# INK-USC/RE-Net

Measured on NVIDIA B200. Metric: rgcn_aggregate_edge_messages_per_sec, higher is better.
Workload: dtype f32

## Files before the change

include/renet_b200.h:

```cpp
#ifndef RENET_B200_H
#define RENET_B200_H

#include <stdint.h>

#ifdef __cplusplus
extern "C" {
#endif

typedef enum {
  RENET_OK = 0,
  RENET_ERR_INVALID_ARG = -1,
  RENET_ERR_CUDA = -2,
  RENET_ERR_NO_DEVICE = -3
} renet_status;

int renet_version(void);
const char* renet_last_error(void);
int64_t renet_launch_count(void);

int renet_set_gemm_engine(int engine);
int renet_get_gemm_engine(void);
int renet_set_weight_generation(int64_t generation);
int renet_set_scratch(void* device_ptr, int64_t bytes);

// ... 12 lines not shown

int renet_selfloop_gemm(const float* H, const int32_t* h_index, const float* Wloop, float* Hout,
                        int64_t N, int32_t d_in, int32_t d_out, void* stream);
int renet_rgcn_gather(const float* H, const int32_t* h_index, const float* W,
                      const int32_t* row_ptr, const int32_t* col_src, const int32_t* col_type,
                      const float* norm, float* Hout,
                      int64_t N, int64_t E, int32_t d_in, int32_t d_out,
                      int32_t num_bases, int32_t R2, int32_t relu, int32_t has_loop, void* stream);
int renet_rgcn_gather_hot(const float* H, const int32_t* h_index, const float* W,
                          const int32_t* row_ptr, const int32_t* col_src, const int32_t* col_type,
                          const float* norm, float* Hout,
                          int64_t N, int64_t E, int32_t d_in, int32_t d_out,
                          int32_t num_bases, int32_t R2, int32_t relu, int32_t has_loop,
                          const int32_t* hot_rel, int32_t n_hot, void* stream);
int renet_debug_stream_timing(void* buffer);

int renet_rgcn_block_bwd(const float* H, const int32_t* h_index,
                         const float* W, const float* Wloop,
                         const int32_t* t_row_ptr, const int32_t* t_col_dst, const int32_t* t_col_type,
                         const int32_t* rel_ptr, const int32_t* rel_src, const int32_t* rel_dst,
                         const float* norm, const float* Hout, const float* dHout,
                         float* dH, float* dW, float* dWloop, float* G_ws,
                         int64_t N, int64_t E, int32_t d_in, int32_t d_out,
                         int32_t num_bases, int32_t R2, int32_t relu, void* stream);

int renet_rgcn_bipartite_bwd(const float* H, const float* W,
                             const int32_t* t_row_ptr, const int32_t* t_col_dst, const int32_t* t_col_type,
                             const int32_t* rel_ptr, const int32_t* rel_src, const int32_t* rel_dst,
                             const float* norm, const float* Hout, const float* dHout,
                             float* dH, float* dW, float* G_ws,
// ... 170 lines not shown
```

renet_b200/_lib.py:

```python
import ctypes
import os

import torch

_HERE = os.path.dirname(os.path.abspath(__file__))
LIB_PATH = os.path.join(_HERE, 'librenet_b200.so')

_vp, _i32, _i64 = ctypes.c_void_p, ctypes.c_int32, ctypes.c_int64

SIGNATURES = {
    'renet_version': (ctypes.c_int, []),
    'renet_last_error': (ctypes.c_char_p, []),
    'renet_launch_count': (_i64, []),
    'renet_set_gemm_engine': (ctypes.c_int, [ctypes.c_int]),
    'renet_get_gemm_engine': (ctypes.c_int, []),
    'renet_set_weight_generation': (ctypes.c_int, [_i64]),
    'renet_set_scratch': (ctypes.c_int, [_vp, _i64]),
    'renet_csr_workspace_bytes': (_i64, [_i64, _i64]),
    'renet_build_csr': (ctypes.c_int, [_vp, _vp, _vp, _i64, _i64, _vp, _vp, _vp, _vp, _vp, _i64, _vp]),
    'renet_rgcn_block_fwd': (ctypes.c_int, [_vp] * 9 + [_i64, _i64, _i32, _i32, _i32, _i32, _i32, _vp]),
    'renet_selfloop_gemm': (ctypes.c_int, [_vp, _vp, _vp, _vp, _i64, _i32, _i32, _vp]),
    'renet_selfloop_gemm_bwd': (ctypes.c_int, [_vp, _vp, _vp, _vp, _vp, _vp, _vp, _i64, _i32, _i32, _vp]),
    'renet_rgcn_gather': (ctypes.c_int, [_vp] * 8 + [_i64, _i64, _i32, _i32, _i32, _i32, _i32, _i32, _vp]),
    'renet_debug_stream_timing': (ctypes.c_int, [_vp]),
    'renet_rgcn_gather_hot': (ctypes.c_int, [_vp] * 8 + [_i64, _i64, _i32, _i32, _i32, _i32, _i32, _i32, _vp, _i32, _vp]),
    'renet_rgcn_block_bwd': (ctypes.c_int, [_vp] * 17 + [_i64, _i64, _i32, _i32, _i32, _i32, _i32, _vp]),
    'renet_rgcn_bipartite_bwd': (ctypes.c_int, [_vp] * 14 + [_i64, _i64, _i64, _i32, _i32, _i32, _i32, _i32, _vp]),
    'renet_readout_subgraph_workspace_bytes': (_i64, [_i64, _i64]),
    'renet_readout_subgraph': (ctypes.c_int, [_vp, _i64, _i64] + [_vp] * 12 + [_i64, _vp]),
    'renet_scatter_add_rows': (ctypes.c_int, [_vp, _vp, _vp, _i64, _i32, _vp]),
    'renet_gru_workspace_bytes': (_i64, [_i64, _i64, _i64, _i32]),
    'renet_gru_fwd': (ctypes.c_int, [_vp] * 11 + [_i32] + [_vp] * 10 + [_i64, _i64, _i64, _i32, _vp, _i64, _vp]),
    'renet_gru_bwd_workspace_bytes': (_i64, [_i64, _i64, _i64, _i32]),
    'renet_gru_bwd': (ctypes.c_int, [_vp] * 11 + [_i32] + [_vp] * 18 + [_i64, _i64, _i64, _i64, _i32, _vp, _vp, _i64, _vp]),
    'renet_gru_dropout_workspace_bytes': (_i64, [_i64, _i64, _i64, _i32]),
    'renet_gru_fwd_dropout': (ctypes.c_int, [_vp] * 12 + [_i32] + [_vp] * 10 + [_i64, _i64, _i64, _i32, ctypes.c_float, ctypes.c_uint64, _vp, _i64, _vp]),
    'renet_gru_bwd_dropout_workspace_bytes': (_i64, [_i64, _i64, _i64, _i32]),
    'renet_gru_bwd_dropout': (ctypes.c_int, [_vp] * 12 + [_i32] + [_vp] * 18 + [_i64, _i64, _i64, _i64, _i32, ctypes.c_float, ctypes.c_uint64, _vp, _vp, _i64, _vp]),
    'renet_dropout_mask': (ctypes.c_int, [ctypes.c_uint64, ctypes.c_uint64, _i64, ctypes.c_float, _vp, _vp]),
# ... 123 lines not shown
```

renet_b200/csrc/api.cu:

```cuda
#include <cub/device/device_radix_sort.cuh>

#include <atomic>
#include <string.h>

#include "common.cuh"

namespace renet {

static thread_local char g_err[512] = "";
static std::atomic<int64_t> g_launches{0};

void set_error(const char* fmt, ...) {
  va_list ap;
  va_start(ap, fmt);
  vsnprintf(g_err, sizeof(g_err), fmt, ap);
  va_end(ap);
}
void count_launch(int n) { g_launches.fetch_add(n, std::memory_order_relaxed); }

int launch_rgcn_gather(const float* H, const int32_t* h_index, const float* W, const int32_t* row_ptr,
                       const int32_t* col_src, const int32_t* col_type, const float* norm, float* Hout,
                       int64_t N, int64_t E, int d_in, int d_out, int nb, int relu, int has_loop,
                       cudaStream_t stream, int R2 = -1, const int32_t* hot_rel = nullptr, int n_hot = 0);
int launch_rgcn_bwd(const float* H, const int32_t* h_index, const float* W, const float* Wloop,
// ... 176 lines not shown
                          int64_t E, int32_t d_in, int32_t d_out, int32_t num_bases, int32_t R2, int32_t relu,
                          int32_t has_loop, const int32_t* hot_rel, int32_t n_hot, void* stream) {
  int rc = check_layer_args("renet_rgcn_gather_hot", H, W, row_ptr, norm, Hout, N, E, d_in, d_out, num_bases, R2);
  if (rc) return rc;
  RENET_CHECK_ARG(E == 0 || (col_src && col_type), "renet_rgcn_gather_hot: null edge arrays");
  RENET_CHECK_ARG(n_hot >= 0 && (n_hot == 0 || hot_rel != nullptr), "renet_rgcn_gather_hot: bad hot-relation list");
  return launch_rgcn_gather(H, h_index, W, row_ptr, col_src, col_type, norm, Hout, N, E, d_in, d_out, num_bases,
                            relu, has_loop, (cudaStream_t)stream, R2, n_hot > 0 ? hot_rel : nullptr, n_hot);
}

int renet_debug_stream_timing(void* buffer) {
  set_stream_debug_buffer(static_cast<long long*>(buffer));
  return RENET_OK;
}

int renet_rgcn_block_fwd(const float* H, const int32_t* h_index, const float* W, const float* Wloop,
                         const int32_t* row_ptr, const int32_t* col_src, const int32_t* col_type,
                         const float* norm, float* Hout, int64_t N, int64_t E, int32_t d_in, int32_t d_out,
                         int32_t num_bases, int32_t R2, int32_t relu, void* stream) {
  int rc = check_layer_args("renet_rgcn_block_fwd", H, W, row_ptr, norm, Hout, N, E, d_in, d_out, num_bases, R2);
  if (rc) return rc;
  RENET_CHECK_ARG(E == 0 || (col_src && col_type), "renet_rgcn_block_fwd: null edge arrays");
  if (N == 0) return RENET_OK;
  if (Wloop != nullptr) {
    rc = sgemm_nn(H, h_index, d_in, Wloop, d_out, Hout, d_out, nullptr, N, d_out, d_in, false, (cudaStream_t)stream);
    if (rc) return rc;
  }
  return launch_rgcn_gather(H, h_index, W, row_ptr, col_src, col_type, norm, Hout, N, E, d_in, d_out, num_bases,
                            relu, Wloop != nullptr, (cudaStream_t)stream, R2);
}
// ... 307 lines not shown
```

renet_b200/csrc/common.cuh:

```cuda
#pragma once
#include <cuda_runtime.h>
#include <stdint.h>
#include <stdio.h>
#include <stdarg.h>

#include "../../include/renet_b200.h"

namespace renet {

void set_error(const char* fmt, ...);
void count_launch(int n = 1);

#define RENET_CHECK_ARG(cond, ...)                  \
  do {                                              \
    if (!(cond)) {                                  \
      ::renet::set_error(__VA_ARGS__);              \
      return RENET_ERR_INVALID_ARG;                 \
    }                                               \
  } while (0)

#define RENET_CHECK_CUDA(expr)                                                        \
  do {                                                                                \
    cudaError_t _e = (expr);                                                          \
    if (_e != cudaSuccess) {                                                          \
// ... 34 lines not shown
}

int sgemm_nn(const float* A, const int32_t* a_index, int64_t lda, const float* B, int64_t ldb, float* C,
             int64_t ldc, const float* bias, int64_t M, int32_t N, int32_t K, bool accumulate,
             cudaStream_t stream);
int sgemm_tn(const float* A, const int32_t* a_index, int64_t lda, const float* B, int64_t ldb, float* C,
             int64_t ldc, int32_t M, int32_t N, int64_t K, bool accumulate, cudaStream_t stream);
int sgemm_nt(const float* A, int64_t lda, const float* B, int64_t ldb, float* C, int64_t ldc,
             int64_t M, int32_t N, int32_t K, bool accumulate, cudaStream_t stream);

int gather_kernel_choice();
constexpr int64_t kStreamMinEdges = 16384;
constexpr int64_t kStreamMinNodes = 16384;
constexpr int64_t kStreamMaxNodes = 98304;
bool gather_use_stream(int64_t E, int64_t N);
void set_stream_debug_buffer(long long* p);

int gemm_mode();
int64_t umma_packed_bytes(int N, int K);
void set_weight_generation(int64_t g);
void* packed_cache_lookup(const void* const* keys, int nkeys, int64_t bytes, bool* hit);
bool umma_shape_ok(int N, int K);
int umma_pack_b(const float* B, int64_t sk, int64_t sn, int N, int K, void* Bp, int tile_offset, cudaStream_t stream);
struct EpiArgs {
  const int32_t* target;
  const float* lse;
  float* pmax;
  float* psum;
  float* tlogit;
  float* dT;
// ... 14 lines not shown
```

renet_b200/csrc/umma_gemm.cu:

```cuda
#include "common.cuh"
#include <mutex>
#include <vector>

#include "umma.cuh"

namespace renet {
namespace {

constexpr int UM = 128;
constexpr int UN = 200;
constexpr int UNP = 208;
constexpr int UKC = 40;
constexpr int USLABS = UKC / 4;
constexpr int UTHREADS = 256;
constexpr int A_SLAB_BYTES = UM * 16;
constexpr int B_SLAB_BYTES = UNP * 16;
constexpr int A_BYTES = USLABS * A_SLAB_BYTES;
constexpr int B_BYTES = USLABS * B_SLAB_BYTES;
constexpr int STAGE_BYTES = 2 * A_BYTES + 2 * B_BYTES;
constexpr int NUM_STAGES = 2;
constexpr int SMEM_BYTES = NUM_STAGES * STAGE_BYTES + 64;
constexpr int TMEM_COLS = 256;

__device__ __forceinline__ uint32_t make_idesc() { return make_idesc_n(UNP); }
// ... 154 lines not shown
  if (warp == 0) {
    asm volatile("tcgen05.dealloc.cta_group::1.sync.aligned.b32 %0, %1;" ::"r"(tmem_base), "n"(TMEM_COLS) : "memory");
  }
}


constexpr int P_BK = 32;
constexpr int P_A_BYTES = UM * 128;
constexpr int P_B_BYTES = UNP * 128;
constexpr int P_B_CHUNK = 2 * P_B_BYTES;
constexpr int P_SMEM = 4 * P_A_BYTES + 2 * P_B_CHUNK + 1024 + 128;

__global__ void __launch_bounds__(256)
umma_pack_b_kernel(const float* __restrict__ B, int64_t sk, int64_t sn, int N, int K, uint8_t* __restrict__ Bp,
                   int n_chunks, int tile_offset) {
  const int nt = blockIdx.x, kc = blockIdx.y;
  const int n0 = nt * UN, k0 = kc * P_BK;
  const int tile_n = min(UN, N - n0);
  uint8_t* dst = Bp + (size_t)((nt + tile_offset) * n_chunks + kc) * P_B_CHUNK;
  for (int task = blockIdx.z * 256 + threadIdx.x; task < UNP * 8; task += 256 * gridDim.z) {
    const int j = task / UNP, n = task % UNP;
    float v[4];
#pragma unroll
    for (int i = 0; i < 4; ++i) {
      const int k = k0 + 4 * j + i;
      v[i] = (n < tile_n && k < K) ? __ldg(B + (int64_t)k * sk + (int64_t)(n0 + n) * sn) : 0.f;
    }
    float4 hi, lo;
    split4(make_float4(v[0], v[1], v[2], v[3]), hi, lo);
    const uint32_t off = sw128_offset(n, j);
// ... 232 lines not shown
  }
  asm volatile("tcgen05.fence::before_thread_sync;" ::: "memory");
  __syncthreads();
  if (warp == 0) {
    asm volatile("tcgen05.dealloc.cta_group::1.sync.aligned.b32 %0, %1;" ::"r"(tmem_base), "n"(512) : "memory");
  }
}

constexpr int SL_PROD_WARPS = 8;
constexpr int SL_PROD = SL_PROD_WARPS * 32;
constexpr int SL_TMA_WARP = 8;
constexpr int SL_MMA_WARP = 9;
constexpr int SL_EPI_WARP0 = 10;
constexpr int SL_THREADS = (SL_EPI_WARP0 + 4) * 32;
constexpr int SL_A_STAGES = 3;
constexpr int SL_B_STAGES = 2;
constexpr int SL_A_STAGE = 2 * P_A_BYTES;
constexpr int SL_EPI_LD = 36;
constexpr int SL_EPI_WARP_BYTES = 32 * SL_EPI_LD * 4;
constexpr int SL_OFF_B = SL_A_STAGES * SL_A_STAGE;
constexpr int SL_OFF_EPI = SL_OFF_B + SL_B_STAGES * P_B_CHUNK;
constexpr int SL_OFF_BAR = SL_OFF_EPI + 4 * SL_EPI_WARP_BYTES;
constexpr int SL_SMEM = SL_OFF_BAR + 128 + 1024;
constexpr int SL_HALF0_N = 112;
static_assert(SL_SMEM <= 227 * 1024, "self-loop kernel: shared memory budget");
static_assert((SL_HALF0_N * 128) % 1024 == 0, "column half must start on a swizzle atom");
constexpr int SL_BAR_A_FULL = 0, SL_BAR_A_EMPTY = 3, SL_BAR_B_FULL = 6, SL_BAR_B_EMPTY = 8, SL_BAR_T_FULL = 10,
              SL_BAR_T_EMPTY = 12, SL_NUM_BARS = 14;

struct SlUnit {
  int64_t row0;
  int col0;
  int n;
};
__device__ __forceinline__ SlUnit sl_unit(int u, int split) {
  SlUnit s;
  if (split) {
    s.row0 = (int64_t)(u >> 1) * UM;
    s.col0 = (u & 1) ? SL_HALF0_N : 0;
    s.n = (u & 1) ? UNP - SL_HALF0_N : SL_HALF0_N;
  } else {
    s.row0 = (int64_t)u * UM;
    s.col0 = 0;
    s.n = UNP;
  }
  return s;
}

template <bool INDEXED>
__global__ void __launch_bounds__(SL_THREADS, 1)
umma_selfloop_kernel(const float* __restrict__ A, const int32_t* __restrict__ a_index, int64_t lda,
                     const uint8_t* __restrict__ Bp, float* __restrict__ C, int64_t ldc, int64_t M, int K, int n_chunks,
                     int n_units, int split) {
  extern __shared__ uint8_t smem_raw[];
  const uint32_t raw = smem_u32(smem_raw);
  uint8_t* smem = smem_raw + ((1024 - (raw & 1023)) & 1023);
  const int tid = threadIdx.x, warp = tid >> 5, lane = tid & 31;
  const uint32_t smem_base = smem_u32(smem);
  const uint32_t bar0 = smem_base + SL_OFF_BAR;
  auto bar = [&](int i) { return bar0 + 8 * i; };
  uint32_t* tmem_slot = reinterpret_cast<uint32_t*>(smem + SL_OFF_BAR + 8 * SL_NUM_BARS);

  if (tid == 0) {
    for (int s = 0; s < SL_A_STAGES; ++s) {
      mbar_init(bar(SL_BAR_A_FULL + s), SL_PROD);
      mbar_init(bar(SL_BAR_A_EMPTY + s), 1);
    }
    for (int s = 0; s < SL_B_STAGES; ++s) {
      mbar_init(bar(SL_BAR_B_FULL + s), 1);
      mbar_init(bar(SL_BAR_B_EMPTY + s), 1);
    }
    for (int a = 0; a < 2; ++a) {
      mbar_init(bar(SL_BAR_T_FULL + a), 1);
      mbar_init(bar(SL_BAR_T_EMPTY + a), 128);
    }
    asm volatile("fence.mbarrier_init.release.cluster;" ::: "memory");
  }
  if (warp == SL_MMA_WARP) {
    asm volatile("tcgen05.alloc.cta_group::1.sync.aligned.shared::cta.b32 [%0], %1;" ::"r"(smem_u32(tmem_slot)), "n"(512)
                 : "memory");
    asm volatile("tcgen05.relinquish_alloc_permit.cta_group::1.sync.aligned;" ::: "memory");
  }
  asm volatile("tcgen05.fence::before_thread_sync;" ::: "memory");
  __syncthreads();
  asm volatile("tcgen05.fence::after_thread_sync;" ::: "memory");
  const uint32_t tmem_base = *tmem_slot;

  const int n_local = (n_units - (int)blockIdx.x + (int)gridDim.x - 1) / (int)gridDim.x;
  const int total = n_local * n_chunks;
  const int last_ks = (K - (n_chunks - 1) * P_BK + 7) / 8;

  if (warp < SL_PROD_WARPS) {
    const int j = tid & 7;
    uint32_t a_off[4];
#pragma unroll
    for (int t = 0; t < 4; ++t) a_off[t] = sw128_offset((tid >> 3) + 32 * t, j);
    const float* rows[4];
    float4 vnext[4];
    auto set_rows = [&](int lu) {
      const SlUnit un = sl_unit((int)blockIdx.x + lu * (int)gridDim.x, split);
#pragma unroll
      for (int t = 0; t < 4; ++t) {
        const int64_t gr = un.row0 + (tid >> 3) + 32 * t;
        rows[t] = nullptr;
        if (gr < M) rows[t] = A + (INDEXED ? (int64_t)__ldg(a_index + gr) : gr) * lda;
      }
    };
    auto load = [&](int c) {
      const int k = c * P_BK + 4 * j;
#pragma unroll
      for (int t = 0; t < 4; ++t) {
        vnext[t] = make_float4(0.f, 0.f, 0.f, 0.f);
        if (rows[t] != nullptr && k < K) vnext[t] = ldg_f4(rows[t] + k);
      }
    };
    set_rows(0);
    load(0);
    for (int it = 0; it < total; ++it) {
      const int s = it % SL_A_STAGES, round = it / SL_A_STAGES;
      float4 v[4];
#pragma unroll
      for (int t = 0; t < 4; ++t) v[t] = vnext[t];
      if (it + 1 < total) {
        const int lu = (it + 1) / n_chunks, c = it + 1 - lu * n_chunks;
        if (c == 0) set_rows(lu);
        load(c);
      }
      if (round > 0) mbar_wait(bar(SL_BAR_A_EMPTY + s), (round - 1) & 1);
      uint8_t* sA_hi = smem + s * SL_A_STAGE;
      uint8_t* sA_lo = sA_hi + P_A_BYTES;
#pragma unroll
      for (int t = 0; t < 4; ++t) {
        float4 hi, lo;
        split4(v[t], hi, lo);
        *reinterpret_cast<float4*>(sA_hi + a_off[t]) = hi;
        *reinterpret_cast<float4*>(sA_lo + a_off[t]) = lo;
      }
      asm volatile("fence.proxy.async.shared::cta;" ::: "memory");
      asm volatile("mbarrier.arrive.shared::cta.b64 _, [%0];" ::"r"(bar(SL_BAR_A_FULL + s)) : "memory");
    }
  } else if (warp == SL_TMA_WARP) {
    if (lane == 0) {
      for (int it = 0; it < total; ++it) {
        const int s = it % SL_B_STAGES, round = it / SL_B_STAGES;
        const int lu = it / n_chunks, c = it - lu * n_chunks;
        const SlUnit un = sl_unit((int)blockIdx.x + lu * (int)gridDim.x, split);
        if (round > 0) mbar_wait(bar(SL_BAR_B_EMPTY + s), (round - 1) & 1);
        const uint32_t full = bar(SL_BAR_B_FULL + s);
        const uint32_t dst = smem_base + SL_OFF_B + s * P_B_CHUNK;
        const uint8_t* src = Bp + (size_t)c * P_B_CHUNK + un.col0 * 128;
        const uint32_t plane = (uint32_t)un.n * 128;
        asm volatile("mbarrier.arrive.expect_tx.shared::cta.b64 _, [%0], %1;" ::"r"(full), "r"(2 * plane) : "memory");
        if (un.n == UNP) {
          asm volatile("cp.async.bulk.shared::cluster.global.mbarrier::complete_tx::bytes [%0], [%1], %2, [%3];" ::"r"(dst),
                       "l"(src), "r"((uint32_t)P_B_CHUNK), "r"(full)
                       : "memory");
        } else {
#pragma unroll
          for (int p = 0; p < 2; ++p)
            asm volatile("cp.async.bulk.shared::cluster.global.mbarrier::complete_tx::bytes [%0], [%1], %2, [%3];" ::"r"(
                             dst + p * P_B_BYTES),
                         "l"(src + p * P_B_BYTES), "r"(plane), "r"(full)
                         : "memory");
        }
      }
    }
    __syncwarp();
  } else if (warp == SL_MMA_WARP) {
    if (lane == 0) {
      int it = 0;
      for (int lu = 0; lu < n_local; ++lu) {
        const int acc = lu & 1;
        const SlUnit un = sl_unit((int)blockIdx.x + lu * (int)gridDim.x, split);
        const uint32_t idesc = make_idesc_n(un.n);
        if (lu >= 2) mbar_wait(bar(SL_BAR_T_EMPTY + acc), ((lu >> 1) - 1) & 1);
        asm volatile("tcgen05.fence::after_thread_sync;" ::: "memory");
        const uint32_t d = tmem_base + acc * 256;
        for (int c = 0; c < n_chunks; ++c, ++it) {
          const int sa = it % SL_A_STAGES, sb = it % SL_B_STAGES;
          mbar_wait(bar(SL_BAR_A_FULL + sa), (it / SL_A_STAGES) & 1);
          mbar_wait(bar(SL_BAR_B_FULL + sb), (it / SL_B_STAGES) & 1);
          asm volatile("tcgen05.fence::after_thread_sync;" ::: "memory");
          const uint32_t a_hi = smem_base + sa * SL_A_STAGE, a_lo = a_hi + P_A_BYTES;
          const uint32_t b_hi = smem_base + SL_OFF_B + sb * P_B_CHUNK, b_lo = b_hi + P_B_BYTES;
          const int nks = (c == n_chunks - 1) ? last_ks : P_BK / 8;
          for (int ks = 0; ks < nks; ++ks) {
            const uint32_t ko = ks * 32;
            const uint64_t dAh = make_desc_sw128(a_hi + ko), dAl = make_desc_sw128(a_lo + ko);
            const uint64_t dBh = make_desc_sw128(b_hi + ko), dBl = make_desc_sw128(b_lo + ko);
            umma_tf32(d, dAh, dBh, idesc, (c | ks) != 0);
            umma_tf32(d, dAl, dBh, idesc, 1);
            umma_tf32(d, dAh, dBl, idesc, 1);
          }
          umma_commit(bar(SL_BAR_A_EMPTY + sa));
          umma_commit(bar(SL_BAR_B_EMPTY + sb));
        }
        umma_commit(bar(SL_BAR_T_FULL + acc));
      }
    }
    __syncwarp();
  } else {
    const int q = warp & 3;
    float* stg = reinterpret_cast<float*>(smem + SL_OFF_EPI + (warp - SL_EPI_WARP0) * SL_EPI_WARP_BYTES);
    for (int lu = 0; lu < n_local; ++lu) {
      const int acc = lu & 1;
      const SlUnit un = sl_unit((int)blockIdx.x + lu * (int)gridDim.x, split);
      const int col_end = min(UN, un.col0 + un.n);
      const int nblk = (un.n + 31) / 32;
      mbar_wait(bar(SL_BAR_T_FULL + acc), (lu >> 1) & 1);
      asm volatile("tcgen05.fence::after_thread_sync;" ::: "memory");
      const uint32_t taddr = tmem_base + acc * 256 + ((uint32_t)(q * 32) << 16);
#pragma unroll 1
      for (int blk = 0; blk < nblk; ++blk) {
        uint32_t v[32];
        asm volatile(
            "tcgen05.ld.sync.aligned.32x32b.x32.b32 "
            "{%0,%1,%2,%3,%4,%5,%6,%7,%8,%9,%10,%11,%12,%13,%14,%15,%16,%17,%18,%19,%20,%21,%22,%23,%24,%25,%26,%27,%28,%29,%30,%31}, [%32];"
            : "=r"(v[0]), "=r"(v[1]), "=r"(v[2]), "=r"(v[3]), "=r"(v[4]), "=r"(v[5]), "=r"(v[6]), "=r"(v[7]), "=r"(v[8]),
              "=r"(v[9]), "=r"(v[10]), "=r"(v[11]), "=r"(v[12]), "=r"(v[13]), "=r"(v[14]), "=r"(v[15]), "=r"(v[16]),
              "=r"(v[17]), "=r"(v[18]), "=r"(v[19]), "=r"(v[20]), "=r"(v[21]), "=r"(v[22]), "=r"(v[23]), "=r"(v[24]),
              "=r"(v[25]), "=r"(v[26]), "=r"(v[27]), "=r"(v[28]), "=r"(v[29]), "=r"(v[30]), "=r"(v[31])
            : "r"(taddr + (uint32_t)(blk * 32)));
        asm volatile("tcgen05.wait::ld.sync.aligned;" ::: "memory");
        if (blk == nblk - 1) {
          asm volatile("tcgen05.fence::before_thread_sync;" ::: "memory");
          asm volatile("mbarrier.arrive.shared::cta.b64 _, [%0];" ::"r"(bar(SL_BAR_T_EMPTY + acc)) : "memory");
        }
#pragma unroll
        for (int i = 0; i < 8; ++i)
          *reinterpret_cast<uint4*>(stg + lane * SL_EPI_LD + 4 * i) = make_uint4(v[4 * i], v[4 * i + 1], v[4 * i + 2], v[4 * i + 3]);
        __syncwarp();
#pragma unroll
        for (int p = 0; p < 8; ++p) {
          const int r = 4 * p + (lane >> 3), c4 = lane & 7;
          const int64_t gr = un.row0 + q * 32 + r;
          const int gc = un.col0 + blk * 32 + 4 * c4;
          if (gr < M && gc < col_end) st_f4(C + gr * ldc + gc, *reinterpret_cast<const float4*>(stg + r * SL_EPI_LD + 4 * c4));
        }
        __syncwarp();
      }
    }
  }
  asm volatile("tcgen05.fence::before_thread_sync;" ::: "memory");
  __syncthreads();
  if (warp == SL_MMA_WARP) {
    asm volatile("tcgen05.dealloc.cta_group::1.sync.aligned.b32 %0, %1;" ::"r"(tmem_base), "n"(512) : "memory");
  }
}

}

static uint8_t* g_scratch = nullptr;
static int64_t g_scratch_bytes = 0;
void set_scratch(void* p, int64_t bytes) { g_scratch = (uint8_t*)p; g_scratch_bytes = p ? bytes : 0; }

namespace {
struct PackEntry {
  int device;
  const void* keys[6];
  int nkeys;
  int64_t bytes;
  void* buf;
  int64_t gen;
};
std::mutex g_pack_mu;
std::vector<PackEntry> g_pack_entries;
int64_t g_weight_generation = -1;
}

// ... 70 lines not shown
#undef RENET_UMMA_LAUNCH
  RENET_CHECK_LAUNCH("umma_gemm_packed_kernel");
  return k_splits;
}

int umma_gemm_prepacked(const float* A, const int32_t* a_index, int64_t lda, const void* Bp, float* C, int64_t ldc,
                        const float* bias, int64_t M, int N, int K, bool accumulate, int batch, int64_t batch_a,
                        int64_t batch_bp, int64_t batch_c, cudaStream_t stream) {
  EpiArgs none{};
  const int r = umma_gemm_prepacked_ex(A, a_index, lda, Bp, C, ldc, bias, M, N, K, accumulate, batch, batch_a, batch_bp, batch_c,
                                       0, none, 1, 0, stream);
  return r < 0 ? r : RENET_OK;
}

static int umma_selfloop(const float* A, const int32_t* a_index, int64_t lda, const void* Bp, float* C, int64_t ldc,
                         int64_t M, int K, cudaStream_t stream) {
  static bool attr = false;
  if (!attr) {
    RENET_CHECK_CUDA(cudaFuncSetAttribute(umma_selfloop_kernel<true>, cudaFuncAttributeMaxDynamicSharedMemorySize, SL_SMEM));
    RENET_CHECK_CUDA(cudaFuncSetAttribute(umma_selfloop_kernel<false>, cudaFuncAttributeMaxDynamicSharedMemorySize, SL_SMEM));
    attr = true;
  }
  static int sm_count[64] = {0};
  int dev = 0;
  RENET_CHECK_CUDA(cudaGetDevice(&dev));
  if (dev < 0 || dev >= 64) dev = 0;
  if (sm_count[dev] == 0) RENET_CHECK_CUDA(cudaDeviceGetAttribute(&sm_count[dev], cudaDevAttrMultiProcessorCount, dev));
  const int sms = sm_count[dev];
  const int64_t tiles = (M + UM - 1) / UM;
  const int split = 2 * tiles <= sms ? 1 : 0;
  const int64_t units = split ? 2 * tiles : tiles;
  RENET_CHECK_ARG(units < (int64_t)1 << 30, "umma_selfloop: too many rows");
  const int grid = (int)(units < sms ? units : sms);
  const int n_chunks = (K + P_BK - 1) / P_BK;
  if (a_index)
    umma_selfloop_kernel<true><<<grid, SL_THREADS, SL_SMEM, stream>>>(A, a_index, lda, (const uint8_t*)Bp, C, ldc, M, K,
                                                                     n_chunks, (int)units, split);
  else
    umma_selfloop_kernel<false><<<grid, SL_THREADS, SL_SMEM, stream>>>(A, a_index, lda, (const uint8_t*)Bp, C, ldc, M, K,
                                                                      n_chunks, (int)units, split);
  RENET_CHECK_LAUNCH("umma_selfloop_kernel");
  return RENET_OK;
}

int umma_gemm_nn_try(const float* A, const int32_t* a_index, int64_t lda, const float* B, int64_t ldb, float* C,
                     int64_t ldc, const float* bias, int64_t M, int32_t N, int32_t K, bool accumulate,
                     cudaStream_t stream) {
  const bool aligned = ((reinterpret_cast<uintptr_t>(A) | reinterpret_cast<uintptr_t>(B) | reinterpret_cast<uintptr_t>(C) |
                         reinterpret_cast<uintptr_t>(bias)) & 15) == 0;
  if (aligned && umma_shape_ok(N, K) && (lda % 4 == 0) && (ldc % 4 == 0) && M >= 64 && g_scratch != nullptr &&
      umma_packed_bytes(N, K) <= g_scratch_bytes && (reinterpret_cast<uintptr_t>(g_scratch) & 127) == 0) {
    bool hit = false;
    const void* keys[4] = {B, reinterpret_cast<const void*>((intptr_t)ldb), reinterpret_cast<const void*>((intptr_t)N),
                           reinterpret_cast<const void*>((intptr_t)K)};
    void* cached = packed_cache_lookup(keys, 4, umma_packed_bytes(N, K), &hit);
    void* Bp = cached ? cached : g_scratch;
    int rc = hit ? 0 : umma_pack_b(B, ldb, 1, N, K, Bp, 0, stream);
    if (rc) return rc;
    if (gemm_mode() == 1 && N == UN && K == UN && bias == nullptr && !accumulate)
      rc = umma_selfloop(A, a_index, lda, Bp, C, ldc, M, K, stream);
    else
      rc = umma_gemm_prepacked(A, a_index, lda, Bp, C, ldc, bias, M, N, K, accumulate, 1, 0, 0, 0, stream);
    return rc ? rc : 1;
  }
  const bool ok = (K % UKC == 0) && K >= UKC && (N % 8 == 0) && (lda % 4 == 0) && (ldb % 4 == 0) && (ldc % 4 == 0) &&
                  M >= 64 && aligned;
  if (!ok) return 0;
  static bool attr_set = false;
  if (!attr_set) {
    cudaError_t e1 = cudaFuncSetAttribute(umma_gemm_nn_kernel<true>, cudaFuncAttributeMaxDynamicSharedMemorySize, SMEM_BYTES);
    cudaError_t e2 = cudaFuncSetAttribute(umma_gemm_nn_kernel<false>, cudaFuncAttributeMaxDynamicSharedMemorySize, SMEM_BYTES);
    if (e1 != cudaSuccess || e2 != cudaSuccess) {
      set_error("cudaFuncSetAttribute(umma_gemm_nn_kernel) failed: %s", cudaGetErrorString(e1 != cudaSuccess ? e1 : e2));
      return RENET_ERR_CUDA;
    }
// ... 18 lines not shown
```

Baseline: 3.809 billion.

## Run self-loop UMMA GEMM as 2-CTA clusters with split B loads and PDL

Converts the self-loop tf32 GEMM kernel to cta_group::2 MMAs over CTA pairs in a cluster. Each CTA loads half of the B columns, and the leader issues the paired MMAs after a peer-ready barrier, so a pair covers a 256-row tile with shared B traffic. It also deepens the B pipeline to four stages, double-buffers the A register prefetch, and adds programmatic dependent launch after the weight pack kernel. Optional per-block timing instrumentation is included. The trade-offs are cross-CTA synchronization cost and fewer work units when M is small.

```diff
diff --git a/include/renet_b200.h b/include/renet_b200.h
--- a/include/renet_b200.h
+++ b/include/renet_b200.h
@@ -50,6 +50,7 @@
                           int32_t num_bases, int32_t R2, int32_t relu, int32_t has_loop,
                           const int32_t* hot_rel, int32_t n_hot, void* stream);
 int renet_debug_stream_timing(void* buffer);
+int renet_debug_selfloop_timing(void* buffer);
 
 int renet_rgcn_block_bwd(const float* H, const int32_t* h_index,
                          const float* W, const float* Wloop,
diff --git a/renet_b200/_lib.py b/renet_b200/_lib.py
--- a/renet_b200/_lib.py
+++ b/renet_b200/_lib.py
@@ -23,6 +23,7 @@
     'renet_selfloop_gemm_bwd': (ctypes.c_int, [_vp, _vp, _vp, _vp, _vp, _vp, _vp, _i64, _i32, _i32, _vp]),
     'renet_rgcn_gather': (ctypes.c_int, [_vp] * 8 + [_i64, _i64, _i32, _i32, _i32, _i32, _i32, _i32, _vp]),
     'renet_debug_stream_timing': (ctypes.c_int, [_vp]),
+    'renet_debug_selfloop_timing': (ctypes.c_int, [_vp]),
     'renet_rgcn_gather_hot': (ctypes.c_int, [_vp] * 8 + [_i64, _i64, _i32, _i32, _i32, _i32, _i32, _i32, _vp, _i32, _vp]),
     'renet_rgcn_block_bwd': (ctypes.c_int, [_vp] * 17 + [_i64, _i64, _i32, _i32, _i32, _i32, _i32, _vp]),
     'renet_rgcn_bipartite_bwd': (ctypes.c_int, [_vp] * 14 + [_i64, _i64, _i64, _i32, _i32, _i32, _i32, _i32, _vp]),
diff --git a/renet_b200/csrc/api.cu b/renet_b200/csrc/api.cu
--- a/renet_b200/csrc/api.cu
+++ b/renet_b200/csrc/api.cu
@@ -214,6 +214,11 @@
   return RENET_OK;
 }
 
+int renet_debug_selfloop_timing(void* buffer) {
+  set_selfloop_debug_buffer(static_cast<long long*>(buffer));
+  return RENET_OK;
+}
+
 int renet_rgcn_block_fwd(const float* H, const int32_t* h_index, const float* W, const float* Wloop,
                          const int32_t* row_ptr, const int32_t* col_src, const int32_t* col_type,
                          const float* norm, float* Hout, int64_t N, int64_t E, int32_t d_in, int32_t d_out,
diff --git a/renet_b200/csrc/common.cuh b/renet_b200/csrc/common.cuh
--- a/renet_b200/csrc/common.cuh
+++ b/renet_b200/csrc/common.cuh
@@ -72,6 +72,7 @@
 constexpr int64_t kStreamMinNodes = 16384;
 constexpr int64_t kStreamMaxNodes = 98304;
 bool gather_use_stream(int64_t E, int64_t N);
+void set_selfloop_debug_buffer(long long* p);
 void set_stream_debug_buffer(long long* p);
 
 int gemm_mode();
diff --git a/renet_b200/csrc/umma_gemm.cu b/renet_b200/csrc/umma_gemm.cu
--- a/renet_b200/csrc/umma_gemm.cu
+++ b/renet_b200/csrc/umma_gemm.cu
@@ -192,6 +192,7 @@
 __global__ void __launch_bounds__(256)
 umma_pack_b_kernel(const float* __restrict__ B, int64_t sk, int64_t sn, int N, int K, uint8_t* __restrict__ Bp,
                    int n_chunks, int tile_offset) {
+  asm volatile("griddepcontrol.launch_dependents;" ::: "memory");
   const int nt = blockIdx.x, kc = blockIdx.y;
   const int n0 = nt * UN, k0 = kc * P_BK;
   const int tile_n = min(UN, N - n0);
@@ -454,45 +455,128 @@
 constexpr int SL_EPI_WARP0 = 10;
 constexpr int SL_THREADS = (SL_EPI_WARP0 + 4) * 32;
 constexpr int SL_A_STAGES = 3;
-constexpr int SL_B_STAGES = 2;
+constexpr int SL_B_STAGES = 4;
 constexpr int SL_A_STAGE = 2 * P_A_BYTES;
+constexpr int SL_B_PLANE = (UNP / 2) * 128;
+constexpr int SL_B_STAGE = 2 * SL_B_PLANE;
 constexpr int SL_EPI_LD = 36;
 constexpr int SL_EPI_WARP_BYTES = 32 * SL_EPI_LD * 4;
 constexpr int SL_OFF_B = SL_A_STAGES * SL_A_STAGE;
-constexpr int SL_OFF_EPI = SL_OFF_B + SL_B_STAGES * P_B_CHUNK;
+constexpr int SL_OFF_EPI = SL_OFF_B + SL_B_STAGES * SL_B_STAGE;
 constexpr int SL_OFF_BAR = SL_OFF_EPI + 4 * SL_EPI_WARP_BYTES;
-constexpr int SL_SMEM = SL_OFF_BAR + 128 + 1024;
+constexpr int SL_SMEM = SL_OFF_BAR + 256 + 1024;
 constexpr int SL_HALF0_N = 112;
 static_assert(SL_SMEM <= 227 * 1024, "self-loop kernel: shared memory budget");
-static_assert((SL_HALF0_N * 128) % 1024 == 0, "column half must start on a swizzle atom");
-constexpr int SL_BAR_A_FULL = 0, SL_BAR_A_EMPTY = 3, SL_BAR_B_FULL = 6, SL_BAR_B_EMPTY = 8, SL_BAR_T_FULL = 10,
-              SL_BAR_T_EMPTY = 12, SL_NUM_BARS = 14;
+static_assert((SL_HALF0_N * 128) % 1024 == 0 && (SL_HALF0_N / 2 * 128) % 1024 == 0 && ((UNP - SL_HALF0_N) / 2 * 128) % 1024 == 0 &&
+                  (UNP / 2 * 128) % 1024 == 0,
+              "every CTA's share of a column range must start on a swizzle atom");
+constexpr int SL_BAR_A_FULL = 0, SL_BAR_A_EMPTY = 3, SL_BAR_B_FULL = 6, SL_BAR_B_EMPTY = 10, SL_BAR_T_FULL = 14,
+              SL_BAR_T_EMPTY = 16, SL_BAR_PEER_FULL = 18, SL_PEER_SLOTS = 4, SL_NUM_BARS = 22;
+static_assert(SL_PEER_SLOTS > SL_A_STAGES, "the peer runs at most SL_A_STAGES items ahead of the leader");
+static_assert(8 * SL_NUM_BARS + 4 <= 256, "barrier area");
 
 struct SlUnit {
   int64_t row0;
   int col0;
   int n;
 };
-__device__ __forceinline__ SlUnit sl_unit(int u, int split) {
+__device__ __forceinline__ SlUnit sl_unit(int u, int split, int rank) {
   SlUnit s;
-  if (split) {
-    s.row0 = (int64_t)(u >> 1) * UM;
-    s.col0 = (u & 1) ? SL_HALF0_N : 0;
-    s.n = (u & 1) ? UNP - SL_HALF0_N : SL_HALF0_N;
-  } else {
-    s.row0 = (int64_t)u * UM;
-    s.col0 = 0;
-    s.n = UNP;
-  }
+  const int64_t pair_row = split ? (u >> 1) : u;
+  s.row0 = pair_row * (2 * UM) + rank * UM;
+  s.col0 = (split && (u & 1)) ? SL_HALF0_N : 0;
+  s.n = split ? ((u & 1) ? UNP - SL_HALF0_N : SL_HALF0_N) : UNP;
   return s;
+}
+
+__device__ __forceinline__ uint32_t sl_cluster_rank() {
+  uint32_t r;
+  asm volatile("mov.u32 %0, %%cluster_ctarank;" : "=r"(r));
+  return r;
+}
+__device__ __forceinline__ uint32_t sl_mapa(uint32_t saddr, uint32_t rank) {
+  uint32_t r;
+  asm volatile("mapa.shared::cluster.u32 %0, %1, %2;" : "=r"(r) : "r"(saddr), "r"(rank));
+  return r;
+}
+__device__ __forceinline__ void sl_arrive_cluster(uint32_t cluster_addr) {
+  asm volatile("mbarrier.arrive.release.cluster.shared::cluster.b64 _, [%0];" ::"r"(cluster_addr) : "memory");
+}
+__device__ __forceinline__ void sl_cluster_sync() {
+  asm volatile("barrier.cluster.arrive.release.aligned;\n\tbarrier.cluster.wait.acquire.aligned;" ::: "memory");
+}
+__device__ __forceinline__ void sl_wait_cluster(uint32_t bar, uint32_t parity) {
+  uint32_t done = 0;
+  for (int spins = 0; !done; ++spins) {
+    asm volatile(
+        "{\n"
+        ".reg .pred p;\n"
+        "mbarrier.try_wait.parity.acquire.cluster.shared::cta.b64 p, [%1], %2;\n"
+        "selp.u32 %0, 1, 0, p;\n"
+        "}\n"
+        : "=r"(done)
+        : "r"(bar), "r"(parity)
+        : "memory");
+    if (spins > (1 << 20)) __trap();
+  }
+}
+__device__ __forceinline__ void umma_tf32_pair(uint32_t tmem_d, uint64_t adesc, uint64_t bdesc, uint32_t idesc, uint32_t accumulate) {
+  asm volatile(
+      "{\n"
+      ".reg .pred p;\n"
+      "setp.ne.b32 p, %4, 0;\n"
+      "tcgen05.mma.cta_group::2.kind::tf32 [%0], %1, %2, %3, p;\n"
+      "}\n" ::"r"(tmem_d), "l"(adesc), "l"(bdesc), "r"(idesc), "r"(accumulate)
+      : "memory");
+}
+__device__ __forceinline__ void umma_commit_pair(uint32_t bar) {
+  asm volatile("tcgen05.commit.cta_group::2.mbarrier::arrive::one.shared::cluster.multicast::cluster.b64 [%0], %1;" ::"r"(bar),
+               "h"((uint16_t)3)
+               : "memory");
+}
+
+constexpr int SL_DBG_SLOTS = 16;
+enum SlDbg {
+  SL_DBG_GT_ENTRY = 0,
+  SL_DBG_GT_EXIT,
+  SL_DBG_CK_ENTRY,
+  SL_DBG_CK_PROLOGUE,
+  SL_DBG_CK_FIRST_A,
+  SL_DBG_CK_FIRST_B,
+  SL_DBG_WAIT_A,
+  SL_DBG_WAIT_B,
+  SL_DBG_WAIT_T,
+  SL_DBG_CK_LAST_COMMIT,
+  SL_DBG_CK_EPI_END,
+  SL_DBG_CK_EXIT,
+  SL_DBG_UNITS,
+  SL_DBG_WAIT_PEER,
+  SL_DBG_SMID,
+  SL_DBG_RANK,
+};
+__device__ __forceinline__ long long sl_clock() { return clock64(); }
+__device__ __forceinline__ long long sl_gtimer() {
+  long long t;
+  asm volatile("mov.u64 %0, %%globaltimer;" : "=l"(t));
+  return t;
 }
 
 template <bool INDEXED>
 __global__ void __launch_bounds__(SL_THREADS, 1)
 umma_selfloop_kernel(const float* __restrict__ A, const int32_t* __restrict__ a_index, int64_t lda,
                      const uint8_t* __restrict__ Bp, float* __restrict__ C, int64_t ldc, int64_t M, int K, int n_chunks,
-                     int n_units, int split) {
+                     int n_units, int split, long long* __restrict__ dbg) {
   extern __shared__ uint8_t smem_raw[];
+  if (dbg != nullptr) {
+    dbg += (size_t)blockIdx.x * SL_DBG_SLOTS;
+    if (threadIdx.x == 0) {
+      dbg[SL_DBG_GT_ENTRY] = sl_gtimer();
+      dbg[SL_DBG_CK_ENTRY] = sl_clock();
+      unsigned smid;
+      asm volatile("mov.u32 %0, %%smid;" : "=r"(smid));
+      dbg[SL_DBG_SMID] = smid;
+    }
+  }
   const uint32_t raw = smem_u32(smem_raw);
   uint8_t* smem = smem_raw + ((1024 - (raw & 1023)) & 1023);
   const int tid = threadIdx.x, warp = tid >> 5, lane = tid & 31;
@@ -500,6 +584,8 @@
   const uint32_t bar0 = smem_base + SL_OFF_BAR;
   auto bar = [&](int i) { return bar0 + 8 * i; };
   uint32_t* tmem_slot = reinterpret_cast<uint32_t*>(smem + SL_OFF_BAR + 8 * SL_NUM_BARS);
+  const int rank = (int)sl_cluster_rank();
+  const int pair = (int)blockIdx.x >> 1, n_pairs = (int)gridDim.x >> 1;
 
   if (tid == 0) {
     for (int s = 0; s < SL_A_STAGES; ++s) {
@@ -512,21 +598,23 @@
     }
     for (int a = 0; a < 2; ++a) {
       mbar_init(bar(SL_BAR_T_FULL + a), 1);
-      mbar_init(bar(SL_BAR_T_EMPTY + a), 128);
-    }
+      mbar_init(bar(SL_BAR_T_EMPTY + a), 2 * 128);
+    }
+    for (int s = 0; s < SL_PEER_SLOTS; ++s) mbar_init(bar(SL_BAR_PEER_FULL + s), 1);
     asm volatile("fence.mbarrier_init.release.cluster;" ::: "memory");
   }
   if (warp == SL_MMA_WARP) {
-    asm volatile("tcgen05.alloc.cta_group::1.sync.aligned.shared::cta.b32 [%0], %1;" ::"r"(smem_u32(tmem_slot)), "n"(512)
+    asm volatile("tcgen05.alloc.cta_group::2.sync.aligned.shared::cta.b32 [%0], %1;" ::"r"(smem_u32(tmem_slot)), "n"(512)
                  : "memory");
-    asm volatile("tcgen05.relinquish_alloc_permit.cta_group::1.sync.aligned;" ::: "memory");
+    asm volatile("tcgen05.relinquish_alloc_permit.cta_group::2.sync.aligned;" ::: "memory");
   }
   asm volatile("tcgen05.fence::before_thread_sync;" ::: "memory");
-  __syncthreads();
+  sl_cluster_sync();
   asm volatile("tcgen05.fence::after_thread_sync;" ::: "memory");
   const uint32_t tmem_base = *tmem_slot;
-
-  const int n_local = (n_units - (int)blockIdx.x + (int)gridDim.x - 1) / (int)gridDim.x;
+  if (dbg != nullptr && tid == 0) dbg[SL_DBG_CK_PROLOGUE] = sl_clock();
+
+  const int n_local = (n_units - pair + n_pairs - 1) / n_pairs;
   const int total = n_local * n_chunks;
   const int last_ks = (K - (n_chunks - 1) * P_BK + 7) / 8;
 
@@ -536,9 +624,8 @@
 #pragma unroll
     for (int t = 0; t < 4; ++t) a_off[t] = sw128_offset((tid >> 3) + 32 * t, j);
     const float* rows[4];
-    float4 vnext[4];
     auto set_rows = [&](int lu) {
-      const SlUnit un = sl_unit((int)blockIdx.x + lu * (int)gridDim.x, split);
+      const SlUnit un = sl_unit(pair + lu * n_pairs, split, rank);
 #pragma unroll
       for (int t = 0; t < 4; ++t) {
         const int64_t gr = un.row0 + (tid >> 3) + 32 * t;
@@ -546,26 +633,22 @@
         if (gr < M) rows[t] = A + (INDEXED ? (int64_t)__ldg(a_index + gr) : gr) * lda;
       }
     };
-    auto load = [&](int c) {
+    auto issue = [&](int item, float4 (&dst)[4]) {
+      const int lu = item / n_chunks, c = item - lu * n_chunks;
+      if (c == 0 && item > 0) set_rows(lu);
       const int k = c * P_BK + 4 * j;
 #pragma unroll
       for (int t = 0; t < 4; ++t) {
-        vnext[t] = make_float4(0.f, 0.f, 0.f, 0.f);
-        if (rows[t] != nullptr && k < K) vnext[t] = ldg_f4(rows[t] + k);
+        dst[t] = make_float4(0.f, 0.f, 0.f, 0.f);
+        if (rows[t] != nullptr && k < K) dst[t] = ldg_f4(rows[t] + k);
       }
     };
-    set_rows(0);
-    load(0);
-    for (int it = 0; it < total; ++it) {
+    auto step = [&](int it, float4 (&buf)[4]) {
       const int s = it % SL_A_STAGES, round = it / SL_A_STAGES;
       float4 v[4];
 #pragma unroll
-      for (int t = 0; t < 4; ++t) v[t] = vnext[t];
-      if (it + 1 < total) {
-        const int lu = (it + 1) / n_chunks, c = it + 1 - lu * n_chunks;
-        if (c == 0) set_rows(lu);
-        load(c);
-      }
+      for (int t = 0; t < 4; ++t) v[t] = buf[t];
+      if (it + 2 < total) issue(it + 2, buf);
       if (round > 0) mbar_wait(bar(SL_BAR_A_EMPTY + s), (round - 1) & 1);
       uint8_t* sA_hi = smem + s * SL_A_STAGE;
       uint8_t* sA_lo = sA_hi + P_A_BYTES;
@@ -578,73 +661,133 @@
       }
       asm volatile("fence.proxy.async.shared::cta;" ::: "memory");
       asm volatile("mbarrier.arrive.shared::cta.b64 _, [%0];" ::"r"(bar(SL_BAR_A_FULL + s)) : "memory");
+    };
+    float4 buf0[4], buf1[4];
+    set_rows(0);
+    issue(0, buf0);
+    if (total > 1) issue(1, buf1);
+    for (int it = 0; it < total; it += 2) {
+      step(it, buf0);
+      if (it + 1 < total) step(it + 1, buf1);
     }
   } else if (warp == SL_TMA_WARP) {
     if (lane == 0) {
+      asm volatile("griddepcontrol.wait;" ::: "memory");
       for (int it = 0; it < total; ++it) {
         const int s = it % SL_B_STAGES, round = it / SL_B_STAGES;
         const int lu = it / n_chunks, c = it - lu * n_chunks;
-        const SlUnit un = sl_unit((int)blockIdx.x + lu * (int)gridDim.x, split);
+        const SlUnit un = sl_unit(pair + lu * n_pairs, split, rank);
         if (round > 0) mbar_wait(bar(SL_BAR_B_EMPTY + s), (round - 1) & 1);
         const uint32_t full = bar(SL_BAR_B_FULL + s);
-        const uint32_t dst = smem_base + SL_OFF_B + s * P_B_CHUNK;
-        const uint8_t* src = Bp + (size_t)c * P_B_CHUNK + un.col0 * 128;
-        const uint32_t plane = (uint32_t)un.n * 128;
-        asm volatile("mbarrier.arrive.expect_tx.shared::cta.b64 _, [%0], %1;" ::"r"(full), "r"(2 * plane) : "memory");
-        if (un.n == UNP) {
-          asm volatile("cp.async.bulk.shared::cluster.global.mbarrier::complete_tx::bytes [%0], [%1], %2, [%3];" ::"r"(dst),
-                       "l"(src), "r"((uint32_t)P_B_CHUNK), "r"(full)
+        const uint32_t dst = smem_base + SL_OFF_B + s * SL_B_STAGE;
+        const uint32_t half = (uint32_t)(un.n / 2) * 128;
+        const uint8_t* src = Bp + (size_t)c * P_B_CHUNK + (size_t)(un.col0 + rank * (un.n / 2)) * 128;
+        asm volatile("mbarrier.arrive.expect_tx.shared::cta.b64 _, [%0], %1;" ::"r"(full), "r"(2 * half) : "memory");
+#pragma unroll
+        for (int p = 0; p < 2; ++p)
+          asm volatile("cp.async.bulk.shared::cluster.global.mbarrier::complete_tx::bytes [%0], [%1], %2, [%3];" ::"r"(
+                           dst + p * SL_B_PLANE),
+                       "l"(src + p * P_B_BYTES), "r"(half), "r"(full)
                        : "memory");
-        } else {
-#pragma unroll
-          for (int p = 0; p < 2; ++p)
-            asm volatile("cp.async.bulk.shared::cluster.global.mbarrier::complete_tx::bytes [%0], [%1], %2, [%3];" ::"r"(
-                             dst + p * P_B_BYTES),
-                         "l"(src + p * P_B_BYTES), "r"(plane), "r"(full)
-                         : "memory");
-        }
       }
     }
     __syncwarp();
   } else if (warp == SL_MMA_WARP) {
-    if (lane == 0) {
+    if (lane == 0 && rank == 0) {
+      long long w_a = 0, w_b = 0, w_t = 0, w_p = 0, t0 = 0;
       int it = 0;
       for (int lu = 0; lu < n_local; ++lu) {
         const int acc = lu & 1;
-        const SlUnit un = sl_unit((int)blockIdx.x + lu * (int)gridDim.x, split);
-        const uint32_t idesc = make_idesc_n(un.n);
-        if (lu >= 2) mbar_wait(bar(SL_BAR_T_EMPTY + acc), ((lu >> 1) - 1) & 1);
+        const SlUnit un = sl_unit(pair + lu * n_pairs, split, rank);
+        const uint32_t idesc = (make_idesc_n(un.n) & ~(0x1Fu << 24)) | ((uint32_t)(2 * UM) >> 4) << 24;
+        if (dbg != nullptr) t0 = sl_clock();
+        if (lu >= 2) sl_wait_cluster(bar(SL_BAR_T_EMPTY + acc), ((lu >> 1) - 1) & 1);
+        if (dbg != nullptr) w_t += sl_clock() - t0;
         asm volatile("tcgen05.fence::after_thread_sync;" ::: "memory");
         const uint32_t d = tmem_base + acc * 256;
         for (int c = 0; c < n_chunks; ++c, ++it) {
           const int sa = it % SL_A_STAGES, sb = it % SL_B_STAGES;
+          if (dbg != nullptr) t0 = sl_clock();
           mbar_wait(bar(SL_BAR_A_FULL + sa), (it / SL_A_STAGES) & 1);
+          if (dbg != nullptr) {
+            const long long t1 = sl_clock();
+            w_a += t1 - t0;
+            if (it == 0) dbg[SL_DBG_CK_FIRST_A] = t1;
+            t0 = t1;
+          }
           mbar_wait(bar(SL_BAR_B_FULL + sb), (it / SL_B_STAGES) & 1);
+          if (dbg != nullptr) {
+            const long long t1 = sl_clock();
+            w_b += t1 - t0;
+            if (it == 0) dbg[SL_DBG_CK_FIRST_B] = t1;
+            t0 = t1;
+          }
+          sl_wait_cluster(bar(SL_BAR_PEER_FULL + it % SL_PEER_SLOTS), (it / SL_PEER_SLOTS) & 1);
+          if (dbg != nullptr) w_p += sl_clock() - t0;
           asm volatile("tcgen05.fence::after_thread_sync;" ::: "memory");
           const uint32_t a_hi = smem_base + sa * SL_A_STAGE, a_lo = a_hi + P_A_BYTES;
-          const uint32_t b_hi = smem_base + SL_OFF_B + sb * P_B_CHUNK, b_lo = b_hi + P_B_BYTES;
+          const uint32_t b_hi = smem_base + SL_OFF_B + sb * SL_B_STAGE, b_lo = b_hi + SL_B_PLANE;
           const int nks = (c == n_chunks - 1) ? last_ks : P_BK / 8;
           for (int ks = 0; ks < nks; ++ks) {
             const uint32_t ko = ks * 32;
             const uint64_t dAh = make_desc_sw128(a_hi + ko), dAl = make_desc_sw128(a_lo + ko);
             const uint64_t dBh = make_desc_sw128(b_hi + ko), dBl = make_desc_sw128(b_lo + ko);
-            umma_tf32(d, dAh, dBh, idesc, (c | ks) != 0);
-            umma_tf32(d, dAl, dBh, idesc, 1);
-            umma_tf32(d, dAh, dBl, idesc, 1);
+            umma_tf32_pair(d, dAh, dBh, idesc, (c | ks) != 0);
+            umma_tf32_pair(d, dAl, dBh, idesc, 1);
+            umma_tf32_pair(d, dAh, dBl, idesc, 1);
           }
-          umma_commit(bar(SL_BAR_A_EMPTY + sa));
-          umma_commit(bar(SL_BAR_B_EMPTY + sb));
+          umma_commit_pair(bar(SL_BAR_A_EMPTY + sa));
+          umma_commit_pair(bar(SL_BAR_B_EMPTY + sb));
         }
-        umma_commit(bar(SL_BAR_T_FULL + acc));
+        umma_commit_pair(bar(SL_BAR_T_FULL + acc));
+      }
+      if (dbg != nullptr) {
+        dbg[SL_DBG_CK_LAST_COMMIT] = sl_clock();
+        dbg[SL_DBG_WAIT_A] = w_a;
+        dbg[SL_DBG_WAIT_B] = w_b;
+        dbg[SL_DBG_WAIT_T] = w_t;
+        dbg[SL_DBG_WAIT_PEER] = w_p;
+        dbg[SL_DBG_UNITS] = n_local;
+        dbg[SL_DBG_RANK] = rank;
+      }
+    } else if (lane == 0) {
+      const uint32_t peer_full0 = sl_mapa(bar(SL_BAR_PEER_FULL), 0);
+      long long w_a = 0, w_b = 0, t0 = 0;
+      for (int it = 0; it < total; ++it) {
+        if (dbg != nullptr) t0 = sl_clock();
+        mbar_wait(bar(SL_BAR_A_FULL + it % SL_A_STAGES), (it / SL_A_STAGES) & 1);
+        if (dbg != nullptr) {
+          const long long t1 = sl_clock();
+          w_a += t1 - t0;
+          if (it == 0) dbg[SL_DBG_CK_FIRST_A] = t1;
+          t0 = t1;
+        }
+        mbar_wait(bar(SL_BAR_B_FULL + it % SL_B_STAGES), (it / SL_B_STAGES) & 1);
+        if (dbg != nullptr) {
+          const long long t1 = sl_clock();
+          w_b += t1 - t0;
+          if (it == 0) dbg[SL_DBG_CK_FIRST_B] = t1;
+        }
+        sl_arrive_cluster(peer_full0 + 8 * (it % SL_PEER_SLOTS));
+      }
+      if (dbg != nullptr) {
+        dbg[SL_DBG_CK_LAST_COMMIT] = sl_clock();
+        dbg[SL_DBG_WAIT_A] = w_a;
+        dbg[SL_DBG_WAIT_B] = w_b;
+        dbg[SL_DBG_WAIT_T] = 0;
+        dbg[SL_DBG_WAIT_PEER] = 0;
+        dbg[SL_DBG_UNITS] = n_local;
+        dbg[SL_DBG_RANK] = rank;
       }
     }
     __syncwarp();
   } else {
     const int q = warp & 3;
     float* stg = reinterpret_cast<float*>(smem + SL_OFF_EPI + (warp - SL_EPI_WARP0) * SL_EPI_WARP_BYTES);
+    const uint32_t t_empty0 = sl_mapa(bar(SL_BAR_T_EMPTY), 0);
     for (int lu = 0; lu < n_local; ++lu) {
       const int acc = lu & 1;
-      const SlUnit un = sl_unit((int)blockIdx.x + lu * (int)gridDim.x, split);
+      const SlUnit un = sl_unit(pair + lu * n_pairs, split, rank);
       const int col_end = min(UN, un.col0 + un.n);
       const int nblk = (un.n + 31) / 32;
       mbar_wait(bar(SL_BAR_T_FULL + acc), (lu >> 1) & 1);
@@ -664,7 +807,7 @@
         asm volatile("tcgen05.wait::ld.sync.aligned;" ::: "memory");
         if (blk == nblk - 1) {
           asm volatile("tcgen05.fence::before_thread_sync;" ::: "memory");
-          asm volatile("mbarrier.arrive.shared::cta.b64 _, [%0];" ::"r"(bar(SL_BAR_T_EMPTY + acc)) : "memory");
+          sl_arrive_cluster(t_empty0 + 8 * acc);
         }
 #pragma unroll
         for (int i = 0; i < 8; ++i)
@@ -680,11 +823,17 @@
         __syncwarp();
       }
     }
+    if (dbg != nullptr && lane == 0) atomicMax(reinterpret_cast<unsigned long long*>(dbg + SL_DBG_CK_EPI_END), (unsigned long long)sl_clock());
   }
   asm volatile("tcgen05.fence::before_thread_sync;" ::: "memory");
-  __syncthreads();
+  sl_cluster_sync();
   if (warp == SL_MMA_WARP) {
-    asm volatile("tcgen05.dealloc.cta_group::1.sync.aligned.b32 %0, %1;" ::"r"(tmem_base), "n"(512) : "memory");
+    asm volatile("tcgen05.fence::after_thread_sync;" ::: "memory");
+    asm volatile("tcgen05.dealloc.cta_group::2.sync.aligned.b32 %0, %1;" ::"r"(tmem_base), "n"(512) : "memory");
+  }
+  if (dbg != nullptr && tid == 0) {
+    dbg[SL_DBG_CK_EXIT] = sl_clock();
+    dbg[SL_DBG_GT_EXIT] = sl_gtimer();
   }
 }
 
@@ -693,6 +842,8 @@
 static uint8_t* g_scratch = nullptr;
 static int64_t g_scratch_bytes = 0;
 void set_scratch(void* p, int64_t bytes) { g_scratch = (uint8_t*)p; g_scratch_bytes = p ? bytes : 0; }
+static long long* g_selfloop_dbg = nullptr;
+void set_selfloop_debug_buffer(long long* p) { g_selfloop_dbg = p; }
 
 namespace {
 struct PackEntry {
@@ -793,31 +944,51 @@
 }
 
 static int umma_selfloop(const float* A, const int32_t* a_index, int64_t lda, const void* Bp, float* C, int64_t ldc,
-                         int64_t M, int K, cudaStream_t stream) {
+                         int64_t M, int K, bool after_pack, cudaStream_t stream) {
   static bool attr = false;
   if (!attr) {
     RENET_CHECK_CUDA(cudaFuncSetAttribute(umma_selfloop_kernel<true>, cudaFuncAttributeMaxDynamicSharedMemorySize, SL_SMEM));
     RENET_CHECK_CUDA(cudaFuncSetAttribute(umma_selfloop_kernel<false>, cudaFuncAttributeMaxDynamicSharedMemorySize, SL_SMEM));
     attr = true;
   }
-  static int sm_count[64] = {0};
+  cudaLaunchAttribute attrs[2];
+  attrs[0].id = cudaLaunchAttributeClusterDimension;
+  attrs[0].val.clusterDim.x = 2;
+  attrs[0].val.clusterDim.y = 1;
+  attrs[0].val.clusterDim.z = 1;
+  attrs[1].id = cudaLaunchAttributeProgrammaticStreamSerialization;
+  attrs[1].val.programmaticStreamSerializationAllowed = 1;
+  cudaLaunchConfig_t cfg = {};
+  cfg.blockDim = dim3(SL_THREADS);
+  cfg.dynamicSmemBytes = SL_SMEM;
+  cfg.stream = stream;
+  cfg.attrs = attrs;
+  cfg.numAttrs = 1;
+  auto kernel = a_index ? umma_selfloop_kernel<true> : umma_selfloop_kernel<false>;
+  static int max_pairs[64] = {0};
   int dev = 0;
   RENET_CHECK_CUDA(cudaGetDevice(&dev));
   if (dev < 0 || dev >= 64) dev = 0;
-  if (sm_count[dev] == 0) RENET_CHECK_CUDA(cudaDeviceGetAttribute(&sm_count[dev], cudaDevAttrMultiProcessorCount, dev));
-  const int sms = sm_count[dev];
-  const int64_t tiles = (M + UM - 1) / UM;
-  const int split = 2 * tiles <= sms ? 1 : 0;
-  const int64_t units = split ? 2 * tiles : tiles;
+  if (max_pairs[dev] == 0) {
+    int sms = 0;
+    RENET_CHECK_CUDA(cudaDeviceGetAttribute(&sms, cudaDevAttrMultiProcessorCount, dev));
+    cfg.gridDim = dim3((unsigned)(sms & ~1));
+    int n = 0;
+    RENET_CHECK_CUDA(cudaOccupancyMaxActiveClusters(&n, umma_selfloop_kernel<true>, &cfg));
+    RENET_CHECK_ARG(n >= 1, "umma_selfloop: no cluster of two CTAs fits on this device");
+    max_pairs[dev] = n;
+  }
+  const int pairs_max = max_pairs[dev];
+  const int64_t pair_rows = (M + 2 * UM - 1) / (2 * UM);
+  const int split = 2 * pair_rows <= pairs_max ? 1 : 0;
+  const int64_t units = split ? 2 * pair_rows : pair_rows;
   RENET_CHECK_ARG(units < (int64_t)1 << 30, "umma_selfloop: too many rows");
-  const int grid = (int)(units < sms ? units : sms);
+  const int pairs = (int)(units < pairs_max ? units : pairs_max);
   const int n_chunks = (K + P_BK - 1) / P_BK;
-  if (a_index)
-    umma_selfloop_kernel<true><<<grid, SL_THREADS, SL_SMEM, stream>>>(A, a_index, lda, (const uint8_t*)Bp, C, ldc, M, K,
-                                                                     n_chunks, (int)units, split);
-  else
-    umma_selfloop_kernel<false><<<grid, SL_THREADS, SL_SMEM, stream>>>(A, a_index, lda, (const uint8_t*)Bp, C, ldc, M, K,
-                                                                      n_chunks, (int)units, split);
+  cfg.gridDim = dim3((unsigned)(2 * pairs));
+  cfg.numAttrs = after_pack ? 2 : 1;
+  RENET_CHECK_CUDA(cudaLaunchKernelEx(&cfg, kernel, A, a_index, lda, (const uint8_t*)Bp, C, ldc, M, K, n_chunks, (int)units,
+                                      split, g_selfloop_dbg));
   RENET_CHECK_LAUNCH("umma_selfloop_kernel");
   return RENET_OK;
 }
@@ -837,7 +1008,7 @@
     int rc = hit ? 0 : umma_pack_b(B, ldb, 1, N, K, Bp, 0, stream);
     if (rc) return rc;
     if (gemm_mode() == 1 && N == UN && K == UN && bias == nullptr && !accumulate)
-      rc = umma_selfloop(A, a_index, lda, Bp, C, ldc, M, K, stream);
+      rc = umma_selfloop(A, a_index, lda, Bp, C, ldc, M, K, !hit, stream);
     else
       rc = umma_gemm_prepacked(A, a_index, lda, Bp, C, ldc, bias, M, N, K, accumulate, 1, 0, 0, 0, stream);
     return rc ? rc : 1;
```

Result: slower. 3.684 billion, median of 6 (-3.3%).
